# cboin1996/avddpg

Measured on AMD Instinct MI355X. Metric: env-steps/sec + DDPG updates/sec, 4096x5-vehicle platoons, higher is better.
Workload: dtype f32-class (fp16 hi+lo operand pairs on the 16-bit matrix cores, f32 accumulate)

## Files before the change

### avddpg_amd/csrc/fsplit.hip

```cpp
#include <type_traits>

#include "fset_common.h"

namespace avd {
namespace fsplit {
using namespace fset;

struct ActorS {
    static constexpr int K = 256, KP = 256, NFT = 8, NKS = 16, LD = 264, NGT = 9, KG = 288;
    static constexpr bool critic = false;
};
struct CriticS {
    static constexpr int K = 304, KP = 320, NFT = 10, NKS = 19, LD = 312, NGT = 10, KG = 320;
    static constexpr bool critic = true;
};
constexpr int NGT_MAX = 10;

template <int I, int N, class F>
__device__ __forceinline__ void static_for(F&& f) {
    if constexpr (I < N) {
        f(std::integral_constant<int, I>{});
        static_for<I + 1, N>(f);
    }
}
// ... 634 lines not shown
#endif
    if (watch >= 0x7f800000u) atomicOr(p.bad, 1);
    if (BOTH) {
#pragma unroll
        for (int o = 1; o < 32; o <<= 1) {
            Dacc += __shfl_xor(Dacc, o), Lacc += __shfl_xor(Lacc, o);
            Dacc2 += __shfl_xor(Dacc2, o), Lacc2 += __shfl_xor(Lacc2, o);
        }
#pragma unroll
        for (int o = 1; o < 64; o <<= 1) gmax = fmaxf(gmax, __shfl_xor(gmax, o));
        if (lane == 0) {
            const long slot = (long)blockIdx.x * 8 + w;
            p.part_m[slot] = gmax;
            p.part_s[slot * 2] = Dacc, p.part_s[slot * 2 + 1] = Lacc;
            p.part_s2[slot * 2] = Dacc2, p.part_s2[slot * 2 + 1] = Lacc2;
        }
    }
}

struct SeedArgs {
    int n_agents, n_sets;
    const float *dmu, *tz;
    float high;
    float *g3, *part_m, *part_s;
};
__global__ __launch_bounds__(NT) void actor_seed_kernel(const SeedArgs p) {
    const int tid = threadIdx.x, w = tid >> 6, lane = tid & 63;
    const int set = blockIdx.x % p.n_sets, j0 = blockIdx.x / p.n_sets, J = gridDim.x / p.n_sets, P = p.n_agents / p.n_sets;
    float gmax = 0.f, D = 0.f;
    for (int pi = j0 + w * J; pi < P; pi += 8 * J) {
        const long ri = (long)(pi * p.n_sets + set) * TILE + lane;
        const float t = p.tz[ri], g = p.dmu[ri] * p.high * (1.f - t * t);
        p.g3[ri] = g;
        gmax = fmaxf(gmax, fabsf(g));
        D += g;
    }
#pragma unroll
    for (int o = 1; o < 64; o <<= 1) gmax = fmaxf(gmax, __shfl_xor(gmax, o)), D += __shfl_xor(D, o);
    if (lane == 0) {
        p.part_m[(long)blockIdx.x * 8 + w] = gmax;
        p.part_s[((long)blockIdx.x * 8 + w) * 2] = D, p.part_s[((long)blockIdx.x * 8 + w) * 2 + 1] = 0.f;
    }
}

__device__ __forceinline__ float set_gscale(const float* part_m, int set, int n_sets, int J, float* red) {
    const int tid = threadIdx.x;
    float m = 0.f;
    for (int i = tid; i < J * 8; i += NT) m = fmaxf(m, part_m[((long)(i >> 3) * n_sets + set) * 8 + (i & 7)]);
#pragma unroll
    for (int o = 1; o < 64; o <<= 1) m = fmaxf(m, __shfl_xor(m, o));
    if ((tid & 63) == 0) red[tid >> 6] = m;
    __syncthreads();
    m = fmaxf(fmaxf(fmaxf(red[0], red[1]), fmaxf(red[2], red[3])), fmaxf(fmaxf(red[4], red[5]), fmaxf(red[6], red[7])));
    int e = 0;
    if (m > 0.f && !not_finite(m)) (void)frexpf(m, &e);
    const int k = e > 100 ? -100 : (e < -100 ? 100 : -e);
    return __uint_as_float(__builtin_amdgcn_readfirstlane(__float_as_uint(ldexpf(1.f, k))));
}

__device__ __forceinline__ unsigned mask_pair(unsigned d, int j, unsigned mj) { return __umul24(d & (0x10001u << j), mj); }
__device__ __forceinline__ void mask_chunk16(unsigned w, int c, unsigned m, uint4& lo, uint4& hi) {
    const unsigned d = w >> (8 * (c & 1));
    lo.x = mask_pair(d, 0, m), lo.y = mask_pair(d, 1, m >> 1), lo.z = mask_pair(d, 2, m >> 2), lo.w = mask_pair(d, 3, m >> 3);
    hi.x = mask_pair(d, 4, m >> 4), hi.y = mask_pair(d, 5, m >> 5), hi.z = mask_pair(d, 6, m >> 6), hi.w = mask_pair(d, 7, m >> 7);
}
__device__ __forceinline__ unsigned mask_one(float g3, bool signed_) { return signed_ && g3 < 0.f ? 0xbc00u : 0x3c00u; }

struct DwArgs {
    NetP net;
    int n_agents, n_sets;
    const float* x;
    const float* act;
    const float* g3;
    const float* part_m;
    const unsigned* sm;
    float* partG;
    int abl;
    unsigned long long* stamp;
};
template <int S, class NET>
__global__ __launch_bounds__(NT) void dw_kernel(const DwArgs p) {
    constexpr int KG = NET::KG, LDZ = 160;
    constexpr int XC = NET::critic ? 2 : 1;
    constexpr bool SGN = !NET::critic;
    __shared__ __attribute__((aligned(16))) unsigned short sgn16[2][TILE];
    __shared__ __attribute__((aligned(16))) f16 smimg[2][TILE * LDZ];
    __shared__ __attribute__((aligned(16))) f16x8 fq[2][TILE * 2];
    __shared__ __attribute__((aligned(16))) f16x8 fa[2][TILE * 2];
    __shared__ float gred[8];
    const int tid = threadIdx.x, w = tid >> 6, lane = tid & 63, r = lane & 31, h = lane >> 5;
    const int set = blockIdx.x % p.n_sets, j0 = blockIdx.x / p.n_sets, J = gridDim.x / p.n_sets, P = p.n_agents / p.n_sets;
    const float gsc = set_gscale(p.part_m, set, p.n_sets, J, gred);
    const f16x8* wf1 = p.net.wf1h + (long)set * NGT_MAX * 64 + lane;
    const int xt = NET::critic ? 8 + (w >> 2) : 8, xrh = NET::critic ? (w >> 1) & 1 : (w >> 2) & 1, xc0 = NET::critic ? 2 * (w & 1) : (w & 3);
    const f16x8 wf0 = wf1[64 * w], wfx = wf1[64 * xt];
    f32x16 G0[4], G1[XC];
    const f32x16 zero16 = {};
#pragma unroll
    for (int c = 0; c < 4; ++c) G0[c] = zero16;
#pragma unroll
    for (int c = 0; c < XC; ++c) G1[c] = zero16;

    const int srow = tid >> 3, sch = tid & 7, frow = tid >> 1, fh = tid & 1;
    unsigned ma = 0, mb = 0;
    float sx[4] = {0.f, 0.f, 0.f, 0.f}, sg = 0.f, sa = 0.f, ga = 0.f, gb = 0.f;
    auto fetch_m = [&](int pl, unsigned& m, float& g) {
        const long ri = (long)(((FSPLIT_ABL(p.abl) & 1) ? j0 : pl) * p.n_sets + set) * TILE + srow;
        m = p.sm[ri * 4 + (sch >> 1)];
        if (NET::critic) g = p.g3[ri];
    };
    auto fetch_x = [&](int pl) {
        if (pl >= P || tid >= 2 * TILE) return;
        const long ri = (long)(pl * p.n_sets + set) * TILE + frow;
        load_x<S>(p.x, ri, sx);
        sg = p.g3[ri];
        if (NET::critic) sa = p.act[ri];
    };
    auto stage = [&](int pl, int buf, unsigned m, float g) {
        if (pl >= P) return;
        uint4* dst = (uint4*)(smimg[buf] + srow * LDZ + 16 * sch);
        mask_chunk16(m, sch, mask_one(g, NET::critic), dst[0], dst[1]);
        if (tid < 2 * TILE) {
            const float g = fabsf(sg) * gsc;
            fq[buf][tid] = make_xg(g * sx[0], g * sx[1], g * sx[2], g * sx[3], g, fh);
            if (NET::critic) fa[buf][tid] = make_xg(g * sa, 0.f, 0.f, 0.f, g, fh);
            if (SGN && fh == 0) sgn16[buf][frow] = sg < 0.f ? 0x8000 : 0;
        }
    };
    const int g4 = lane >> 4, q = (lane & 15) >> 2, pp = lane & 3;
    typedef _Float16 f16x4 __attribute__((ext_vector_type(4)));
    auto read_tr = [&](const f16* at) {
        return __builtin_bit_cast(f16x4, __builtin_amdgcn_ds_read_tr16_b64_v4bf16((__attribute__((address_space(3))) bf16x4*)at));
    };
    auto read_b = [&](int buf, int e, int s, f16x8 (&bfr)[4]) {
#pragma unroll
        for (int c = 0; c < 4; ++c)
#pragma unroll
            for (int hf = 0; hf < 2; ++hf) {
                const int R0 = 32 * e + 16 * s + 8 * hf + 4 * (g4 >> 1);
                const f16x4 t = read_tr(smimg[buf] + (R0 + q) * LDZ + 32 * c + 16 * (g4 & 1) + 4 * pp);
#pragma unroll
                for (int j = 0; j < 4; ++j) bfr[c][4 * hf + j] = t[j];
            }
    };
    auto split16e = [&](const f32x16& p1, unsigned (&qh)[8], unsigned (&ql)[8], int buf, int e) {
        if (FSPLIT_ABL(p.abl) & 4) {
#pragma unroll
            for (int m = 0; m < 8; ++m) qh[m] = __float_as_uint(p1[2 * m]), ql[m] = __float_as_uint(p1[2 * m + 1]);
            return;
        }
#pragma unroll
        for (int m = 0; m < 8; ++m) split2h(relu(p1[2 * m]), relu(p1[2 * m + 1]), qh[m], ql[m]);
        if (SGN) {
#pragma unroll
            for (int qd = 0; qd < 4; ++qd) {
                const uint2 sw = *(const uint2*)((const unsigned*)sgn16[buf] + 16 * e + 4 * qd + 2 * h);
                qh[2 * qd] ^= sw.x, ql[2 * qd] ^= sw.x, qh[2 * qd + 1] ^= sw.y, ql[2 * qd + 1] ^= sw.y;
            }
        }
    };
    auto compute = [&](int buf) {
        unsigned ah[8], al[8], bh[8], bl[8];
        split16e(mfmah(fq[buf][r * 2 + h], wf0, zero16), ah, al, buf, 0);
        __builtin_amdgcn_sched_barrier(0);
        {
            const f32x16 p1 = mfmah(fq[buf][(32 + r) * 2 + h], wf0, zero16);
#pragma unroll
            for (int s = 0; s < 2; ++s) {
                f16x8 bfr[4];
                read_b(buf, 0, s, bfr);
                const f16x8 hi = fragh(ah[4 * s], ah[4 * s + 1], ah[4 * s + 2], ah[4 * s + 3]);
                const f16x8 lo = fragh(al[4 * s], al[4 * s + 1], al[4 * s + 2], al[4 * s + 3]);
#pragma unroll
                for (int c = 0; c < 4; ++c) G0[c] = mfmah(hi, bfr[c], G0[c]), G0[c] = mfmah(lo, bfr[c], G0[c]);
            }
            split16e(p1, bh, bl, buf, 1);
            __builtin_amdgcn_sched_group_barrier(0x008, 1, 0);
#pragma unroll
            for (int s = 0; s < 2; ++s) {
                __builtin_amdgcn_sched_group_barrier(0x100, 8, 0);
#pragma unroll
                for (int i = 0; i < 8; ++i) {
                    __builtin_amdgcn_sched_group_barrier(0x008, 1, 0);
                    __builtin_amdgcn_sched_group_barrier(0x002, SGN ? 4 : 3, 0);
                }
            }
            __builtin_amdgcn_sched_barrier(0);
        }
        {
            const f16x8 xin = NET::critic ? fa[buf][(32 * xrh + r) * 2 + h] : fq[buf][(32 * xrh + r) * 2 + h];
            const f32x16 px = mfmah(xin, wfx, zero16);
#pragma unroll
            for (int s = 0; s < 2; ++s) {
                f16x8 bfr[4];
                read_b(buf, 1, s, bfr);
                const f16x8 hi = fragh(bh[4 * s], bh[4 * s + 1], bh[4 * s + 2], bh[4 * s + 3]);
                const f16x8 lo = fragh(bl[4 * s], bl[4 * s + 1], bl[4 * s + 2], bl[4 * s + 3]);
#pragma unroll
                for (int c = 0; c < 4; ++c) G0[c] = mfmah(hi, bfr[c], G0[c]), G0[c] = mfmah(lo, bfr[c], G0[c]);
            }
            split16e(px, ah, al, buf, xrh);
            __builtin_amdgcn_sched_group_barrier(0x008, 1, 0);
#pragma unroll
            for (int s = 0; s < 2; ++s) {
                __builtin_amdgcn_sched_group_barrier(0x100, 8, 0);
#pragma unroll
                for (int i = 0; i < 8; ++i) {
                    __builtin_amdgcn_sched_group_barrier(0x008, 1, 0);
                    __builtin_amdgcn_sched_group_barrier(0x002, SGN ? 4 : 3, 0);
                }
            }
            __builtin_amdgcn_sched_barrier(0);
        }
#pragma unroll
        for (int s = 0; s < 2; ++s) {
            const f16x8 hi = fragh(ah[4 * s], ah[4 * s + 1], ah[4 * s + 2], ah[4 * s + 3]);
            const f16x8 lo = fragh(al[4 * s], al[4 * s + 1], al[4 * s + 2], al[4 * s + 3]);
#pragma unroll
            for (int c = 0; c < XC; ++c) {
                f16x8 bx;
#pragma unroll
                for (int hf = 0; hf < 2; ++hf) {
                    const int R0 = 32 * xrh + 16 * s + 8 * hf + 4 * (g4 >> 1);
                    const f16x4 t = read_tr(smimg[buf] + (R0 + q) * LDZ + 32 * (xc0 + c) + 16 * (g4 & 1) + 4 * pp);
#pragma unroll
                    for (int j = 0; j < 4; ++j) bx[4 * hf + j] = t[j];
                }
                G1[c] = mfmah(hi, bx, G1[c]);
                G1[c] = mfmah(lo, bx, G1[c]);
            }
        }
    };
    if (j0 < P) fetch_m(j0, ma, ga);
    fetch_x(j0);
    if (j0 + J < P) fetch_m(j0 + J, mb, gb);
    stage(j0, 0, ma, ga);
    __syncthreads();
#ifdef AVD_STAMP
    unsigned long long tacc[4] = {0, 0, 0, 0}, tlast = __builtin_amdgcn_s_memtime();
#define STAMP(i) { const unsigned long long t_ = __builtin_amdgcn_s_memtime(); tacc[i] += t_ - tlast; tlast = t_; }
#else
#define STAMP(i)
#endif
    for (int pi = j0; pi < P; pi += 2 * J) {
        fetch_x(pi + J);
        if (pi + 2 * J < P) fetch_m(pi + 2 * J, ma, ga);
        STAMP(0);
        compute(0);
        STAMP(1);
        stage(pi + J, 1, mb, gb);
        STAMP(2);
        if (!(FSPLIT_ABL(p.abl) & 2)) __syncthreads();
        STAMP(3);
        if (pi + J < P) {
            fetch_x(pi + 2 * J);
            if (pi + 3 * J < P) fetch_m(pi + 3 * J, mb, gb);
            STAMP(0);
            compute(1);
            STAMP(1);
            stage(pi + 2 * J, 0, ma, ga);
            STAMP(2);
            if (!(FSPLIT_ABL(p.abl) & 2)) __syncthreads();
            STAMP(3);
        }
    }
#ifdef AVD_STAMP
    if (p.stamp && blockIdx.x == 16 && lane == 0)
        for (int i = 0; i < 4; ++i) p.stamp[w * 8 + i] = tacc[i];
#endif
    const float dsc = 1.f / (gsc * S1);
    float* comb = (float*)&smimg[0][0];
    const int cidx = NET::critic ? 2 * (w >> 2) + (w & 1) : (w & 3);
    if (xrh == 1) {
#pragma unroll
        for (int c = 0; c < XC; ++c)
#pragma unroll
            for (int k = 0; k < 16; ++k) comb[((cidx * XC + c) * 16 + k) * 64 + lane] = G1[c][k];
    }
    __syncthreads();
#pragma unroll
    for (int c = 0; c < 4; ++c) {
        float* dst = p.partG + ((long)blockIdx.x * KG + 32 * w) * H2 + 32 * c + r;
#pragma unroll
        for (int k = 0; k < 16; ++k) dst[(long)acc_row(k, h) * H2] = G0[c][k] * dsc;
    }
    if (xrh == 0) {
#pragma unroll
        for (int c = 0; c < XC; ++c) {
            float* dst = p.partG + ((long)blockIdx.x * KG + 32 * xt) * H2 + 32 * (xc0 + c) + r;
#pragma unroll
            for (int k = 0; k < 16; ++k) dst[(long)acc_row(k, h) * H2] = (G1[c][k] + comb[((cidx * XC + c) * 16 + k) * 64 + lane]) * dsc;
        }
    }
}

struct DxArgs {
    NetP net;
    int n_agents, n_sets;
    const f16x8* xfh;
    const float* act;
    int L_cWa, L_cba;
    const float* g3;
    const float* part_m;
    const unsigned* sm;
    int unsigned_mask;
    float* partV;
    int abl;
    unsigned long long* stamp;
};
template <int S, class NET>
__global__ __launch_bounds__(NT) void dx_kernel(const DxArgs p) {
    constexpr int KP = NET::KP, LDZ = 136;
    constexpr float VSH = 1.f / 32.f;
    __shared__ __attribute__((aligned(16))) f16 smimg[2][TILE * LDZ];
    __shared__ __attribute__((aligned(16))) f16 xt[2][2][32 * 32];
    __shared__ __attribute__((aligned(16))) float g3s[2][TILE];
    __shared__ float gred[8];
    const int tid = threadIdx.x, w = __builtin_amdgcn_readfirstlane(tid >> 6), lane = tid & 63, r = lane & 31, h = lane >> 5, ft = w;
    const int set = blockIdx.x % p.n_sets, j0 = blockIdx.x / p.n_sets, J = gridDim.x / p.n_sets, P = p.n_agents / p.n_sets;
    const f32x16 zero16 = {};
    const float gsc = set_gscale(p.part_m, set, p.n_sets, J, gred);
    f16x8 wch[8], wcl[8];
    {
        const long at = ((long)set * KP + 32 * ft + r) * H2 + 8 * h;
#pragma unroll
        for (int s = 0; s < 8; ++s) wch[s] = *(const f16x8*)(p.net.Wchi + at + 16 * s), wcl[s] = *(const f16x8*)(p.net.Wclo + at + 16 * s);
    }
    const float swc = __uint_as_float(__builtin_amdgcn_readfirstlane(__float_as_uint(p.net.vec[(long)set * VEC + 2 * H2 + 2])));
    const float gv = gsc * VSH, vs = gsc * swc * VSH;
    const f16x8 wf = p.net.wf1h[((long)set * NGT_MAX + ft) * 64 + lane];
    f32x16 V = zero16;
    for (int i = tid; i < 2 * 2 * 32 * 32; i += NT) {
        const int k = (i >> 5) & 31;
        (&xt[0][0][0])[i] = (f16)(k == 8 ? 1.f : 0.f);
    }
    const int srow = tid >> 3, sch = tid & 7;
    unsigned dm = 0;
    float gn = 0.f, gs = 0.f;
    auto fetch = [&](int agent) {
        if (FSPLIT_ABL(p.abl) & 1) agent = j0 * p.n_sets + set;
        dm = p.sm[((long)agent * TILE + srow) * 4 + (sch >> 1)];
        if (NET::critic) gs = p.g3[(long)agent * TILE + srow];
        if (tid < TILE) gn = p.g3[(long)agent * TILE + tid];
    };
    auto stage = [&](int buf) {
        uint4* dst = (uint4*)(smimg[buf] + srow * LDZ + 16 * sch);
        mask_chunk16(dm, sch, mask_one(gs, NET::critic), dst[0], dst[1]);
        if (tid < TILE) g3s[buf][tid] = (p.unsigned_mask ? gn : fabsf(gn)) * gv;
    };
    f16x8 xfn0 = {}, xfn1 = {};
    auto fetch_x = [&](int agent) {
        xfn0 = p.xfh[((long)agent * TILE + r) * 2 + h];
        xfn1 = p.xfh[((long)agent * TILE + 32 + r) * 2 + h];
    };
    auto stage_x = [&](int buf) {
        if (w < 2 && h == 0) {
            f16x8 src = xfn0;
            if (w == 1) src = xfn1;
            asm volatile("" : "+v"(src));
#pragma unroll
            for (int k = 0; k < 8; ++k) xt[buf][w][k * 32 + r] = src[k];
        }
    };
    __syncthreads();
    if (j0 < P) fetch(j0 * p.n_sets + set), fetch_x(j0 * p.n_sets + set), stage(0), stage_x(0);
    __syncthreads();
#ifdef AVD_STAMP
    unsigned long long dacc[4] = {0, 0, 0, 0}, dlast = __builtin_amdgcn_s_memtime();
#define DXSTAMP(i) { const unsigned long long t_ = __builtin_amdgcn_s_memtime(); dacc[i] += t_ - dlast; dlast = t_; }
#else
#define DXSTAMP(i)
#endif
    int buf = 0;
    for (int pi = j0; pi < P; pi += J, buf ^= 1) {
        const bool more = pi + J < P;
        const f16x8 xf[2] = {xfn0, xfn1};
        if (more) fetch((pi + J) * p.n_sets + set), fetch_x((pi + J) * p.n_sets + set);
        DXSTAMP(0);
        auto read_a = [&](int e, f16x8 (&smf)[8]) {
            const f16* arow = smimg[buf] + (32 * e + r) * LDZ + 8 * h;
#pragma unroll
            for (int s = 0; s < 8; ++s) smf[s] = *(const f16x8*)(arow + 16 * s);
        };
        typedef _Float16 f16x4 __attribute__((ext_vector_type(4)));
        auto read_img = [&](const f16* img, f16x8 (&xb)[2]) {
#pragma unroll
            for (int s = 0; s < 2; ++s) {
                const f16x4 lo = *(const f16x4*)(img + r * 32 + 16 * s + 4 * h);
                const f16x4 hi = *(const f16x4*)(img + r * 32 + 16 * s + 8 + 4 * h);
#pragma unroll
                for (int j = 0; j < 4; ++j) xb[s][j] = lo[j], xb[s][4 + j] = hi[j];
            }
        };
        auto backward = [&](int e, const f32x16& dc, const f32x16& p1, unsigned (&vh)[8], unsigned (&vl)[8]) {
            if (FSPLIT_ABL(p.abl) & 4) {
#pragma unroll
                for (int m = 0; m < 8; ++m) vh[m] = __float_as_uint(dc[2 * m]) ^ __float_as_uint(p1[2 * m]), vl[m] = __float_as_uint(dc[2 * m + 1]);
                return;
            }
#pragma unroll
            for (int g = 0; g < 4; ++g) {
                const float4 gq = *(const float4*)(&g3s[buf][32 * e + 8 * g + 4 * h]);
                const float gg[4] = {gq.x, gq.y, gq.z, gq.w};
                float dm[4];
#pragma unroll
                for (int j = 0; j < 4; ++j) {
                    const int k = 4 * g + j;
                    dm[j] = p1[k] > 0.f ? dc[k] * gg[j] : 0.f;
                }
                split2h(dm[0], dm[1], vh[2 * g], vl[2 * g]);
                split2h(dm[2], dm[3], vh[2 * g + 1], vl[2 * g + 1]);
            }
        };
        f16x8 smf[8], xb0[2], xb1[2];
        unsigned vh0[8], vl0[8], vh1[8], vl1[8];
        read_a(0, smf);
        f32x16 dc0 = zero16;
#pragma unroll
        for (int s = 0; s < 8; ++s) dc0 = mfmah(smf[s], wch[s], dc0), dc0 = mfmah(smf[s], wcl[s], dc0);
        const f32x16 p10 = mfmah(xf[0], wf, zero16);
        __builtin_amdgcn_sched_barrier(0);
        read_a(1, smf);
        read_img(xt[buf][0], xb0);
        f32x16 dc1 = zero16;
#pragma unroll
        for (int s = 0; s < 8; ++s) dc1 = mfmah(smf[s], wch[s], dc1), dc1 = mfmah(smf[s], wcl[s], dc1);
        const f32x16 p11 = mfmah(xf[1], wf, zero16);
        backward(0, dc0, p10, vh0, vl0);
        __builtin_amdgcn_sched_group_barrier(0x100, 12, 0);
#pragma unroll
        for (int i = 0; i < 17; ++i) {
            __builtin_amdgcn_sched_group_barrier(0x008, 1, 0);
            __builtin_amdgcn_sched_group_barrier(0x002, 5, 0);
            __builtin_amdgcn_sched_group_barrier(0x100, 1, 0);
        }
        __builtin_amdgcn_sched_barrier(0);
        read_img(xt[buf][1], xb1);
#pragma unroll
        for (int s = 0; s < 2; ++s) {
            V = mfmah(fragh(vh0[4 * s], vh0[4 * s + 1], vh0[4 * s + 2], vh0[4 * s + 3]), xb0[s], V);
            V = mfmah(fragh(vl0[4 * s], vl0[4 * s + 1], vl0[4 * s + 2], vl0[4 * s + 3]), xb0[s], V);
        }
        backward(1, dc1, p11, vh1, vl1);
#pragma unroll
        for (int s = 0; s < 2; ++s) {
            V = mfmah(fragh(vh1[4 * s], vh1[4 * s + 1], vh1[4 * s + 2], vh1[4 * s + 3]), xb1[s], V);
            V = mfmah(fragh(vl1[4 * s], vl1[4 * s + 1], vl1[4 * s + 2], vl1[4 * s + 3]), xb1[s], V);
        }
        DXSTAMP(1);
        if (more) stage(buf ^ 1), stage_x(buf ^ 1);
        DXSTAMP(2);
        if (!(FSPLIT_ABL(p.abl) & 2)) __syncthreads();
        DXSTAMP(3);
    }
#ifdef AVD_STAMP
    if (p.stamp && blockIdx.x == 16 && lane == 0)
        for (int i = 0; i < 4; ++i) p.stamp[w * 8 + i] = dacc[i];
#endif
    const float ivs = 1.f / vs;
    if (r < 16) {
        float* pv = p.partV + ((long)blockIdx.x * KP + 32 * ft) * 16 + r;
#pragma unroll
        for (int k = 0; k < 16; ++k) pv[(long)acc_row(k, h) * 16] = V[k] * ivs;
    }
}

template <int S>
__global__ __launch_bounds__(NT) void dxa_kernel(const DxArgs p) {
    typedef CriticS NET;
    constexpr int KP = NET::KP;
    constexpr float VSH = 1.f / 32.f;
    __shared__ __attribute__((aligned(16))) float ga[8][2][2][32];
    __shared__ float comb[8][64][2];
    __shared__ float gred[8];
    const int tid = threadIdx.x, w = __builtin_amdgcn_readfirstlane(tid >> 6), lane = tid & 63, r = lane & 31, h = lane >> 5;
    const int rh = w & 1, ftl = (w >> 1) & 1, par = w >> 2;
    const int set = blockIdx.x % p.n_sets, j0 = blockIdx.x / p.n_sets, J = gridDim.x / p.n_sets, P = p.n_agents / p.n_sets;
    const f32x16 zero16 = {};
    const int ft = 8 + ftl, f = 32 * ftl + r;
    const float gsc = set_gscale(p.part_m, set, p.n_sets, J, gred);
    f16x8 wch[8], wcl[8];
    {
        const long at = ((long)set * KP + 32 * ft + r) * H2 + 8 * h;
#pragma unroll
        for (int s = 0; s < 8; ++s) wch[s] = *(const f16x8*)(p.net.Wchi + at + 16 * s), wcl[s] = *(const f16x8*)(p.net.Wclo + at + 16 * s);
    }
    const float swc = __uint_as_float(__builtin_amdgcn_readfirstlane(__float_as_uint(p.net.vec[(long)set * VEC + 2 * H2 + 2])));
    const float gv = gsc * VSH, vs = gsc * swc * VSH;
    const float* th = p.net.th + (long)set * p.net.th_stride;
    const float wa = f < HA ? th[p.L_cWa + f] : 0.f, ba = f < HA ? th[p.L_cba + f] : 0.f;
    float Sa = 0.f, Sb = 0.f;
    const int ntile = j0 < P ? (P - j0 + J - 1) / J : 0;
    uint4 mA = {}, mB = {};
    float gA = 0.f, aA = 0.f, gB = 0.f, aB = 0.f;
#define DXA_FETCH(k_, m_, g_, a_)                                                                                   \
    {                                                                                                               \
        const long r0_ = (long)((j0 + (k_) * J) * p.n_sets + set) * TILE + 32 * rh;                                 \
        m_ = *(const uint4*)(p.sm + (r0_ + r) * 4);                                                                 \
        g_ = p.g3[r0_ + r], a_ = p.act[r0_ + r];                                                                    \
    }
#define DXA_PUT(buf_, g_, a_)                                                                                       \
    {                                                                                                               \
        if (h == 0) ga[w][buf_][0][r] = fabsf(g_) * gv, ga[w][buf_][1][r] = a_;                                     \
        __builtin_amdgcn_fence(__ATOMIC_RELEASE, "wavefront");                                                      \
        __builtin_amdgcn_wave_barrier();                                                                            \
    }
    auto unit = [&](int buf, const uint4 mw, float g) {
        f32x16 dc = zero16;
        const unsigned m = mask_one(g, true);
        const unsigned mwt[4] = {mw.x >> (4 * h), mw.y >> (4 * h), mw.z >> (4 * h), mw.w >> (4 * h)};
#pragma unroll
        for (int s = 0; s < 8; ++s) {
            const unsigned d = mwt[s >> 1] >> (8 * (s & 1));
            const f16x8 af = fragh(mask_pair(d, 0, m), mask_pair(d, 1, m >> 1), mask_pair(d, 2, m >> 2), mask_pair(d, 3, m >> 3));
            dc = mfmah(af, wch[s], dc), dc = mfmah(af, wcl[s], dc);
        }
        float sa = 0.f, sb = 0.f;
#pragma unroll
        for (int q = 0; q < 4; ++q) {
            const float4 gq = *(const float4*)(&ga[w][buf][0][8 * q + 4 * h]), aq = *(const float4*)(&ga[w][buf][1][8 * q + 4 * h]);
            const float gg[4] = {gq.x, gq.y, gq.z, gq.w}, av[4] = {aq.x, aq.y, aq.z, aq.w};
#pragma unroll
            for (int j = 0; j < 4; ++j) {
                const float m = fmaf(av[j], wa, ba) > 0.f ? dc[4 * q + j] * gg[j] : 0.f;
                sa = fmaf(m, av[j], sa);
                sb += m;
            }
        }
        Sa += sa, Sb += sb;
        __builtin_amdgcn_fence(__ATOMIC_ACQ_REL, "wavefront");
        __builtin_amdgcn_wave_barrier();
    };
    if (par < ntile) DXA_FETCH(par, mA, gA, aA);
    if (par + 2 < ntile) DXA_FETCH(par + 2, mB, gB, aB);
    for (int k = par; k < ntile; k += 4) {
        DXA_PUT(0, gA, aA);
// ... 53 lines not shown
        pl.Whi[i] = take(sizeof(f16) * (size_t)n_sets * H2 * K), pl.Wlo[i] = take(sizeof(f16) * (size_t)n_sets * H2 * K);
        pl.vec[i] = take(sizeof(float) * (size_t)n_sets * VEC);
        pl.wf1h[i] = take(16 * (size_t)n_sets * NGT_MAX * 64);
        if (i < 2) pl.Wchi[i] = take(sizeof(f16) * (size_t)n_sets * KP * H2), pl.Wclo[i] = take(sizeof(f16) * (size_t)n_sets * KP * H2);
    }
    pl.wap = take(4 * (size_t)n_sets * 48);
    const size_t rows = (size_t)n_agents * TILE;
    pl.a2 = take(4 * rows), pl.y = take(4 * rows), pl.mu = take(4 * rows), pl.dmu = take(4 * rows), pl.g3 = take(4 * rows);
    pl.sm = take(16 * rows);
    pl.sma = take(16 * rows);
    pl.tz = take(4 * rows);
    pl.t1p = take(2 * 4 * (size_t)n_sets * CriticS::K * H2), pl.s2raw = take(2 * 4 * (size_t)n_sets * H2);
    pl.xfs = take(32 * rows), pl.xfs2 = take(32 * rows);
    for (int i = 0; i < 2; ++i) {
        const int KP = i ? CriticS::KP : ActorS::KP, KG = i ? CriticS::KG : ActorS::KG;
        pl.partM[i] = take(4 * (size_t)pl.grid * 8);
        pl.partV[i] = take(4 * (size_t)pl.grid * KP * 16);
        pl.partG[i] = take(4 * (size_t)pl.grid * KG * H2);
    }
    for (int i = 0; i < 3; ++i) pl.partHs[i] = take(4 * (size_t)pl.grid * 8 * 2);
    pl.bad = take(sizeof(int) + sizeof(unsigned) * 4 * (size_t)n_sets * 2);
    pl.total = o;
    return pl;
}
static int check_shape(const avd_mlp_layout* L, int n_agents, int n_sets, const char* who) {
    AVD_REQUIRE(L, "%s: null layout", who);
    if (L->H1 != H1 || L->H2 != H2 || L->Ha != HA || L->A != 1 || (L->S != 3 && L->S != 4) || L->B != TILE) {
        set_error("%s: serves the reference widths only (layer1 256, layer2 128, action layer 48, A = 1, S in {3, 4}, B = 64); "
                  "got H1=%d H2=%d Ha=%d A=%d S=%d B=%d (avd_learn_shared_bf16 takes other widths)",
                  who, L->H1, L->H2, L->Ha, L->A, L->S, L->B);
        return AVD_E_UNSUPPORTED;
    }
    AVD_REQUIRE(n_sets > 0 && n_sets <= 64 && n_agents > 0 && n_agents % n_sets == 0, "%s: n_agents=%d n_sets=%d", who, n_agents,
                n_sets);
    return AVD_OK;
}

enum Phase { PH_CRITIC = 1, PH_ACTOR = 2, PH_BOTH = 3 };
template <int S>
static int run(int phases, const avd_mlp_layout& L, int n_agents, int n_sets, const float* theta, const float* stats, const float* theta_t,
               const float* stats_t, const float* s, const float* a, const float* r, const float* s2, const float* aw, float gamma,
               float high, float* grads, float* losses, unsigned char* ws, const Plan& pl, hipStream_t st) {
    PrepArgs pa;
    pa.L = L, pa.S = S, pa.theta = theta, pa.stats = stats, pa.theta_t = theta_t, pa.stats_t = stats_t;
    pa.wap = (unsigned*)(ws + pl.wap), pa.bad = (int*)(ws + pl.bad), pa.smax = (unsigned*)(ws + pl.bad + sizeof(int));
    NetP net[4];
    for (int i = 0; i < 4; ++i) {
        const bool critic = i & 1, target = i >= 2;
        pa.Whi[i] = (f16*)(ws + pl.Whi[i]), pa.Wlo[i] = (f16*)(ws + pl.Wlo[i]), pa.vec[i] = (float*)(ws + pl.vec[i]);
        pa.wf1h[i] = (f16x8*)(ws + pl.wf1h[i]);
        pa.Wchi[i] = i < 2 ? (f16*)(ws + pl.Wchi[i]) : nullptr, pa.Wclo[i] = i < 2 ? (f16*)(ws + pl.Wclo[i]) : nullptr;
        NetP& n = net[i];
        n.th = (target ? theta_t : theta) + (critic ? L.actor_size : 0), n.th_stride = L.theta_size;
        n.Whi = pa.Whi[i], n.Wlo = pa.Wlo[i], n.Wchi = pa.Wchi[i], n.Wclo = pa.Wclo[i], n.wf1h = pa.wf1h[i], n.vec = pa.vec[i];
        n.wap = pa.wap;
    }
    const int P = n_agents / n_sets;
    const float inv_n = 1.0f / ((float)P * TILE);
    const long nrows = (long)n_agents * TILE;
    f16x8 *xfs = (f16x8*)(ws + pl.xfs), *xfs2 = (f16x8*)(ws + pl.xfs2);
    int* bad = (int*)(ws + pl.bad);
    float *a2 = (float*)(ws + pl.a2), *y = (float*)(ws + pl.y), *mu = (float*)(ws + pl.mu), *dmu = (float*)(ws + pl.dmu);
    float* g3 = (float*)(ws + pl.g3);
    unsigned *sm = (unsigned*)(ws + pl.sm), *sma = (unsigned*)(ws + pl.sma);
    auto F = [&](size_t off) { return (float*)(ws + off); };
    const dim3 grid(pl.grid), block(NT);
    HeadArgs h;
    h.n_agents = n_agents, h.n_sets = n_sets, h.gamma = gamma, h.high = high, h.inv_n = inv_n, h.aw = aw, h.sm = sm, h.g3 = g3, h.dmu = dmu;
    h.act2 = nullptr, h.part_s2 = nullptr, h.stamp = nullptr, h.bad = bad, h.part_m = nullptr, h.tz = F(pl.tz), h.abl = 0;
    if (const char* e = AVD_DIAG_ENV("FSPLIT_ABL")) h.abl = atoi(e);
    auto head = [&](auto kern, int ni, const f16x8* x, const float* act, const float* rr, const float* yin, float* out, float* part_s) {
        h.net = net[ni], h.xf = x, h.act = act, h.r = rr, h.yin = yin, h.out = out, h.part_s = part_s;
        hipLaunchKernelGGL(kern, grid, block, 0, st, h);
    };
    DwArgs dw;
    dw.n_agents = n_agents, dw.n_sets = n_sets, dw.sm = sm, dw.g3 = g3, dw.x = s, dw.stamp = nullptr, dw.abl = 0;
    if (const char* e = AVD_DIAG_ENV("FSPLIT_ABL")) dw.abl = atoi(e);
#ifdef AVD_STAMP
    static unsigned long long* d_stamp = nullptr;
    if (!d_stamp) (void)hipMalloc(&d_stamp, 128 * 8);
    dw.stamp = d_stamp;
#endif
    DxArgs dx;
    dx.n_agents = n_agents, dx.n_sets = n_sets, dx.sm = sm, dx.g3 = g3, dx.xfh = xfs, dx.stamp = nullptr, dx.L_cWa = dx.L_cba = 0, dx.unsigned_mask = 0;
    dx.abl = dw.abl;
#ifdef AVD_STAMP
    dx.stamp = d_stamp;
#endif
    FinArgs fa;
    fa.L = L, fa.n_sets = n_sets, fa.J = pl.J, fa.S = S, fa.nrh = 1, fa.theta = theta, fa.stats = stats, fa.grads = grads, fa.losses = losses;
    fa.inv_n = inv_n, fa.partLa = F(pl.partHs[2]), fa.bad = bad;
    for (int i = 0; i < 2; ++i)
        fa.partH[i] = nullptr, fa.partHs[i] = F(pl.partHs[i]), fa.partU[i] = nullptr, fa.partV[i] = F(pl.partV[i]),
        fa.partG[i] = F(pl.partG[i]), fa.c3[i] = F(pl.vec[i]);
    fa.t1_from_g[0] = fa.t1_from_g[1] = 1, fa.t1p = F(pl.t1p), fa.s2raw = F(pl.s2raw);
    if (phases & PH_CRITIC) {
        if (hipMemsetAsync(ws + pl.bad, 0, sizeof(int) + sizeof(unsigned) * 4 * (size_t)n_sets * 2, st) != hipSuccess)
            return check_launch("avd_learn_set_split: memset");
        hipLaunchKernelGGL(scale_kernel, dim3(4, n_sets, SCALE_SLICES), dim3(256), 0, st, pa);
        hipLaunchKernelGGL(prep_kernel, dim3(H2, 4, n_sets), dim3(320), 0, st, pa);
        hipLaunchKernelGGL(prep1_kernel, dim3(NGT_MAX, 4, n_sets), dim3(64), 0, st, pa);
        PackArgs pk;
        pk.x[0] = s, pk.extra[0] = a, pk.outh[0] = xfs, pk.x[1] = s2, pk.extra[1] = r, pk.outh[1] = xfs2, pk.rows = nrows, pk.bad = bad;
        hipLaunchKernelGGL(pack_x_kernel<S>, dim3((unsigned)((2 * nrows + 255) / 256), 2), dim3(256), 0, st, pk);
        head(head_kernel<S, ActorS, OUT_TANH>, 2, xfs2, nullptr, nullptr, nullptr, a2, nullptr);
        head(head_kernel<S, CriticS, OUT_TD>, 3, xfs2, a2, r, nullptr, y, nullptr);
        h.sm = sma;
        head(head_kernel<S, ActorS, OUT_TANH_SAVE>, 0, xfs, nullptr, nullptr, nullptr, mu, nullptr);
        h.sm = sm;
        h.act2 = mu, h.part_s2 = F(pl.partHs[2]), h.part_m = F(pl.partM[1]);
        head(head_kernel<S, CriticS, HEAD_BOTH>, 1, xfs, a, nullptr, y, nullptr, F(pl.partHs[1]));
        dw.net = net[1], dw.act = a, dw.partG = F(pl.partG[1]), dw.part_m = F(pl.partM[1]);
        hipLaunchKernelGGL((dw_kernel<S, CriticS>), grid, block, 0, st, dw);
        dx.net = net[1], dx.partV = F(pl.partV[1]), dx.act = a, dx.part_m = F(pl.partM[1]);
        hipLaunchKernelGGL((dx_kernel<S, CriticS>), grid, block, 0, st, dx);
        dx.L_cWa = L.cWa, dx.L_cba = L.cba;
        hipLaunchKernelGGL((dxa_kernel<S>), grid, block, 0, st, dx);
        if (phases == PH_CRITIC) launch_finalize(fa, st, 1, 1);
    }
    if (phases & PH_ACTOR) {
        SeedArgs sd;
        sd.n_agents = n_agents, sd.n_sets = n_sets, sd.dmu = dmu, sd.tz = F(pl.tz), sd.high = high, sd.g3 = g3, sd.part_m = F(pl.partM[0]),
        sd.part_s = F(pl.partHs[0]);
        hipLaunchKernelGGL(actor_seed_kernel, grid, block, 0, st, sd);
        dw.sm = sma, dx.sm = sma;
        dw.net = net[0], dw.act = nullptr, dw.partG = F(pl.partG[0]), dw.part_m = F(pl.partM[0]);
        hipLaunchKernelGGL((dw_kernel<S, ActorS>), grid, block, 0, st, dw);
        dx.net = net[0], dx.partV = F(pl.partV[0]), dx.act = nullptr, dx.part_m = F(pl.partM[0]), dx.L_cWa = dx.L_cba = 0, dx.unsigned_mask = 1;
        hipLaunchKernelGGL((dx_kernel<S, ActorS>), grid, block, 0, st, dx);
        if (phases == PH_ACTOR) launch_finalize(fa, st, 0, 1);
        else launch_finalize(fa, st, 0, 2);
    }
    return check_launch("avd_learn_set_split");
}

}
}

using namespace avd;

namespace avd { namespace fsplit {
constexpr long MFMA_PER_TILE = 2 * (200 + 238 + 200 + 314)
                               + 8 * (2 + 32 + 1 + 2 * 2 * 2)
                               + 8 * (2 + 32 + 1 + 2 * 1 * 2)
                               + 2 * 8 * (32 + 2 + 8)
                               + 4 * 16;
static_assert(MFMA_PER_TILE == 3296, "update DESIGN.md 3.4 and the count above together");
}}
extern "C" int avd_learn_set_split_mfma_count(const avd_mlp_layout* lay, int n_agents, int n_sets, unsigned long long* mfma_32x32x16) {
    int rc = fsplit::check_shape(lay, n_agents, n_sets, "avd_learn_set_split_mfma_count");
    if (rc) return rc;
    AVD_REQUIRE(mfma_32x32x16, "avd_learn_set_split_mfma_count: null pointer");
    *mfma_32x32x16 = (unsigned long long)fsplit::MFMA_PER_TILE * (unsigned long long)n_agents;
    return AVD_OK;
}

extern "C" int avd_learn_set_split_workspace(const avd_mlp_layout* lay, int n_agents, int n_sets, size_t* bytes) {
    int rc = fsplit::check_shape(lay, n_agents, n_sets, "avd_learn_set_split_workspace");
    if (rc) return rc;
    AVD_REQUIRE(bytes, "avd_learn_set_split_workspace: null pointer");
    *bytes = fsplit::make_plan(n_agents, n_sets).total;
    return AVD_OK;
}

static int split_entry(int phases, const char* who, const avd_mlp_layout* lay, int n_agents, int n_sets, const float* theta, const float* stats,
                       const float* theta_t, const float* stats_t, const float* s, const float* a, const float* r, const float* s2,
                       const float* agent_weight, float gamma, float high, float* grads, float* losses, void* workspace,
                       size_t workspace_bytes, void* stream) {
    int rc = fsplit::check_shape(lay, n_agents, n_sets, who);
    if (rc) return rc;
    const bool cr = phases & fsplit::PH_CRITIC;
    AVD_REQUIRE(theta && stats && s && grads && workspace && (!cr || (theta_t && stats_t && a && r && s2)), "%s: null pointer", who);
    const fsplit::Plan pl = fsplit::make_plan(n_agents, n_sets);
    AVD_REQUIRE(workspace_bytes >= pl.total, "%s: workspace %zu B < %zu B", who, workspace_bytes, pl.total);
    if (cr && hipMemsetAsync(grads, 0, sizeof(float) * (size_t)n_sets * lay->theta_size, (hipStream_t)stream) != hipSuccess)
        return check_launch("avd_learn_set_split: hipMemsetAsync(grads)");
    if (lay->S == 4)
        return fsplit::run<4>(phases, *lay, n_agents, n_sets, theta, stats, theta_t, stats_t, s, a, r, s2, agent_weight, gamma, high, grads,
                              losses, (unsigned char*)workspace, pl, (hipStream_t)stream);
    return fsplit::run<3>(phases, *lay, n_agents, n_sets, theta, stats, theta_t, stats_t, s, a, r, s2, agent_weight, gamma, high, grads, losses,
                          (unsigned char*)workspace, pl, (hipStream_t)stream);
}

extern "C" int avd_learn_set_split_f16x3(const avd_mlp_layout* lay, int n_agents, int n_sets, const float* theta, const float* stats,
                                          const float* theta_t, const float* stats_t, const float* s, const float* a, const float* r,
                                          const float* s2, const float* agent_weight, float gamma, float high, float* grads,
                                          float* losses, void* workspace, size_t workspace_bytes, void* stream) {
    return split_entry(fsplit::PH_BOTH, "avd_learn_set_split_f16x3", lay, n_agents, n_sets, theta, stats, theta_t, stats_t, s, a, r, s2,
                       agent_weight, gamma, high, grads, losses, workspace, workspace_bytes, stream);
}

extern "C" int avd_learn_set_split_bf16x3(const avd_mlp_layout* lay, int n_agents, int n_sets, const float* theta, const float* stats,
                                          const float* theta_t, const float* stats_t, const float* s, const float* a, const float* r,
                                          const float* s2, const float* agent_weight, float gamma, float high, float* grads,
                                          float* losses, void* workspace, size_t workspace_bytes, void* stream) {
    return avd_learn_set_split_f16x3(lay, n_agents, n_sets, theta, stats, theta_t, stats_t, s, a, r, s2, agent_weight, gamma, high, grads,
                                     losses, workspace, workspace_bytes, stream);
}

extern "C" int avd_learn_set_split_critic(const avd_mlp_layout* lay, int n_agents, int n_sets, const float* theta, const float* stats,
                                          const float* theta_t, const float* stats_t, const float* s, const float* a, const float* r,
                                          const float* s2, const float* agent_weight, float gamma, float high, float* grads,
                                          float* losses, void* workspace, size_t workspace_bytes, void* stream) {
    return split_entry(fsplit::PH_CRITIC, "avd_learn_set_split_critic", lay, n_agents, n_sets, theta, stats, theta_t, stats_t, s, a, r, s2,
                       agent_weight, gamma, high, grads, losses, workspace, workspace_bytes, stream);
}

extern "C" int avd_learn_set_split_actor(const avd_mlp_layout* lay, int n_agents, int n_sets, const float* theta, const float* stats,
                                         const float* s, float high, float* grads, void* workspace, size_t workspace_bytes, void* stream) {
    return split_entry(fsplit::PH_ACTOR, "avd_learn_set_split_actor", lay, n_agents, n_sets, theta, stats, nullptr, nullptr, s, nullptr, nullptr,
                       nullptr, nullptr, 0.f, high, grads, nullptr, workspace, workspace_bytes, stream);
// ... 2 lines not shown
```

Measured before the change: 2.019 million.

## Software-pipeline dx kernel across tiles and fold actor sign into mask staging

The dx kernel is restructured so the second half of each tile's backward pass and V-product run overlapped with the next tile's dc products. Staging now uses a three-slot ring for xt/g3s, with a one-ahead prefetch of mask and x data. In dw, the per-row sign XOR on the split operands is removed and the sign is instead folded into the staged mask image (signed ±1 mask for the actor). Mask staging for the next buffer is moved inside compute, with scheduling hints interleaving it with the MFMAs. Costs are more shared memory, more complex prologue/epilogue logic, and a sign-convention change whose correctness depends on mask_one semantics.

```diff
diff --git a/avddpg_amd/csrc/fsplit.hip b/avddpg_amd/csrc/fsplit.hip
--- a/avddpg_amd/csrc/fsplit.hip
+++ b/avddpg_amd/csrc/fsplit.hip
@@ -740,8 +740,6 @@
 __global__ __launch_bounds__(NT) void dw_kernel(const DwArgs p) {
     constexpr int KG = NET::KG, LDZ = 160;
     constexpr int XC = NET::critic ? 2 : 1;
-    constexpr bool SGN = !NET::critic;
-    __shared__ __attribute__((aligned(16))) unsigned short sgn16[2][TILE];
     __shared__ __attribute__((aligned(16))) f16 smimg[2][TILE * LDZ];
     __shared__ __attribute__((aligned(16))) f16x8 fq[2][TILE * 2];
     __shared__ __attribute__((aligned(16))) f16x8 fa[2][TILE * 2];
@@ -765,7 +763,7 @@
     auto fetch_m = [&](int pl, unsigned& m, float& g) {
         const long ri = (long)(((FSPLIT_ABL(p.abl) & 1) ? j0 : pl) * p.n_sets + set) * TILE + srow;
         m = p.sm[ri * 4 + (sch >> 1)];
-        if (NET::critic) g = p.g3[ri];
+        g = p.g3[ri];
     };
     auto fetch_x = [&](int pl) {
         if (pl >= P || tid >= 2 * TILE) return;
@@ -774,15 +772,16 @@
         sg = p.g3[ri];
         if (NET::critic) sa = p.act[ri];
     };
-    auto stage = [&](int pl, int buf, unsigned m, float g) {
+    auto stage_m = [&](int buf, unsigned m, float g) {
+        uint4* dst = (uint4*)(smimg[buf] + srow * LDZ + 16 * sch);
+        mask_chunk16(m, sch, mask_one(g, true), dst[0], dst[1]);
+    };
+    auto stage_x = [&](int pl, int buf) {
         if (pl >= P) return;
-        uint4* dst = (uint4*)(smimg[buf] + srow * LDZ + 16 * sch);
-        mask_chunk16(m, sch, mask_one(g, NET::critic), dst[0], dst[1]);
         if (tid < 2 * TILE) {
             const float g = fabsf(sg) * gsc;
             fq[buf][tid] = make_xg(g * sx[0], g * sx[1], g * sx[2], g * sx[3], g, fh);
             if (NET::critic) fa[buf][tid] = make_xg(g * sa, 0.f, 0.f, 0.f, g, fh);
-            if (SGN && fh == 0) sgn16[buf][frow] = sg < 0.f ? 0x8000 : 0;
         }
     };
     const int g4 = lane >> 4, q = (lane & 15) >> 2, pp = lane & 3;
@@ -801,7 +800,7 @@
                 for (int j = 0; j < 4; ++j) bfr[c][4 * hf + j] = t[j];
             }
     };
-    auto split16e = [&](const f32x16& p1, unsigned (&qh)[8], unsigned (&ql)[8], int buf, int e) {
+    auto split16e = [&](const f32x16& p1, unsigned (&qh)[8], unsigned (&ql)[8]) {
         if (FSPLIT_ABL(p.abl) & 4) {
 #pragma unroll
             for (int m = 0; m < 8; ++m) qh[m] = __float_as_uint(p1[2 * m]), ql[m] = __float_as_uint(p1[2 * m + 1]);
@@ -809,17 +808,10 @@
         }
 #pragma unroll
         for (int m = 0; m < 8; ++m) split2h(relu(p1[2 * m]), relu(p1[2 * m + 1]), qh[m], ql[m]);
-        if (SGN) {
-#pragma unroll
-            for (int qd = 0; qd < 4; ++qd) {
-                const uint2 sw = *(const uint2*)((const unsigned*)sgn16[buf] + 16 * e + 4 * qd + 2 * h);
-                qh[2 * qd] ^= sw.x, ql[2 * qd] ^= sw.x, qh[2 * qd + 1] ^= sw.y, ql[2 * qd + 1] ^= sw.y;
-            }
-        }
-    };
-    auto compute = [&](int buf) {
+    };
+    auto compute = [&](int buf, unsigned m, float g) {
         unsigned ah[8], al[8], bh[8], bl[8];
-        split16e(mfmah(fq[buf][r * 2 + h], wf0, zero16), ah, al, buf, 0);
+        split16e(mfmah(fq[buf][r * 2 + h], wf0, zero16), ah, al);
         __builtin_amdgcn_sched_barrier(0);
         {
             const f32x16 p1 = mfmah(fq[buf][(32 + r) * 2 + h], wf0, zero16);
@@ -832,7 +824,7 @@
 #pragma unroll
                 for (int c = 0; c < 4; ++c) G0[c] = mfmah(hi, bfr[c], G0[c]), G0[c] = mfmah(lo, bfr[c], G0[c]);
             }
-            split16e(p1, bh, bl, buf, 1);
+            split16e(p1, bh, bl);
             __builtin_amdgcn_sched_group_barrier(0x008, 1, 0);
 #pragma unroll
             for (int s = 0; s < 2; ++s) {
@@ -840,7 +832,7 @@
 #pragma unroll
                 for (int i = 0; i < 8; ++i) {
                     __builtin_amdgcn_sched_group_barrier(0x008, 1, 0);
-                    __builtin_amdgcn_sched_group_barrier(0x002, SGN ? 4 : 3, 0);
+                    __builtin_amdgcn_sched_group_barrier(0x002, 3, 0);
                 }
             }
             __builtin_amdgcn_sched_barrier(0);
@@ -857,7 +849,7 @@
 #pragma unroll
                 for (int c = 0; c < 4; ++c) G0[c] = mfmah(hi, bfr[c], G0[c]), G0[c] = mfmah(lo, bfr[c], G0[c]);
             }
-            split16e(px, ah, al, buf, xrh);
+            split16e(px, ah, al);
             __builtin_amdgcn_sched_group_barrier(0x008, 1, 0);
 #pragma unroll
             for (int s = 0; s < 2; ++s) {
@@ -865,11 +857,12 @@
 #pragma unroll
                 for (int i = 0; i < 8; ++i) {
                     __builtin_amdgcn_sched_group_barrier(0x008, 1, 0);
-                    __builtin_amdgcn_sched_group_barrier(0x002, SGN ? 4 : 3, 0);
+                    __builtin_amdgcn_sched_group_barrier(0x002, 3, 0);
                 }
             }
             __builtin_amdgcn_sched_barrier(0);
         }
+        stage_m(buf ^ 1, m, g);
 #pragma unroll
         for (int s = 0; s < 2; ++s) {
             const f16x8 hi = fragh(ah[4 * s], ah[4 * s + 1], ah[4 * s + 2], ah[4 * s + 3]);
@@ -888,11 +881,19 @@
                 G1[c] = mfmah(lo, bx, G1[c]);
             }
         }
+        __builtin_amdgcn_sched_group_barrier(0x100, 4 * XC, 0);
+#pragma unroll
+        for (int i = 0; i < 4 * XC; ++i) {
+            __builtin_amdgcn_sched_group_barrier(0x008, 1, 0);
+            __builtin_amdgcn_sched_group_barrier(0x002, 6, 0);
+        }
+        __builtin_amdgcn_sched_group_barrier(0x200, 2, 0);
+        __builtin_amdgcn_sched_barrier(0);
     };
     if (j0 < P) fetch_m(j0, ma, ga);
     fetch_x(j0);
     if (j0 + J < P) fetch_m(j0 + J, mb, gb);
-    stage(j0, 0, ma, ga);
+    stage_m(0, ma, ga), stage_x(j0, 0);
     __syncthreads();
 #ifdef AVD_STAMP
     unsigned long long tacc[4] = {0, 0, 0, 0}, tlast = __builtin_amdgcn_s_memtime();
@@ -904,9 +905,9 @@
         fetch_x(pi + J);
         if (pi + 2 * J < P) fetch_m(pi + 2 * J, ma, ga);
         STAMP(0);
-        compute(0);
+        compute(0, mb, gb);
         STAMP(1);
-        stage(pi + J, 1, mb, gb);
+        stage_x(pi + J, 1);
         STAMP(2);
         if (!(FSPLIT_ABL(p.abl) & 2)) __syncthreads();
         STAMP(3);
@@ -914,9 +915,9 @@
             fetch_x(pi + 2 * J);
             if (pi + 3 * J < P) fetch_m(pi + 3 * J, mb, gb);
             STAMP(0);
-            compute(1);
+            compute(1, ma, ga);
             STAMP(1);
-            stage(pi + 2 * J, 0, ma, ga);
+            stage_x(pi + 2 * J, 0);
             STAMP(2);
             if (!(FSPLIT_ABL(p.abl) & 2)) __syncthreads();
             STAMP(3);
@@ -961,7 +962,6 @@
     const float* g3;
     const float* part_m;
     const unsigned* sm;
-    int unsigned_mask;
     float* partV;
     int abl;
     unsigned long long* stamp;
@@ -971,8 +971,8 @@
     constexpr int KP = NET::KP, LDZ = 136;
     constexpr float VSH = 1.f / 32.f;
     __shared__ __attribute__((aligned(16))) f16 smimg[2][TILE * LDZ];
-    __shared__ __attribute__((aligned(16))) f16 xt[2][2][32 * 32];
-    __shared__ __attribute__((aligned(16))) float g3s[2][TILE];
+    __shared__ __attribute__((aligned(16))) f16 xt[3][2][32 * 32];
+    __shared__ __attribute__((aligned(16))) float g3s[3][TILE];
     __shared__ float gred[8];
     const int tid = threadIdx.x, w = __builtin_amdgcn_readfirstlane(tid >> 6), lane = tid & 63, r = lane & 31, h = lane >> 5, ft = w;
     const int set = blockIdx.x % p.n_sets, j0 = blockIdx.x / p.n_sets, J = gridDim.x / p.n_sets, P = p.n_agents / p.n_sets;
@@ -988,128 +988,160 @@
     const float gv = gsc * VSH, vs = gsc * swc * VSH;
     const f16x8 wf = p.net.wf1h[((long)set * NGT_MAX + ft) * 64 + lane];
     f32x16 V = zero16;
-    for (int i = tid; i < 2 * 2 * 32 * 32; i += NT) {
+    for (int i = tid; i < 3 * 2 * 32 * 32; i += NT) {
         const int k = (i >> 5) & 31;
         (&xt[0][0][0])[i] = (f16)(k == 8 ? 1.f : 0.f);
     }
     const int srow = tid >> 3, sch = tid & 7;
     unsigned dm = 0;
     float gn = 0.f, gs = 0.f;
-    auto fetch = [&](int agent) {
-        if (FSPLIT_ABL(p.abl) & 1) agent = j0 * p.n_sets + set;
-        dm = p.sm[((long)agent * TILE + srow) * 4 + (sch >> 1)];
-        if (NET::critic) gs = p.g3[(long)agent * TILE + srow];
-        if (tid < TILE) gn = p.g3[(long)agent * TILE + tid];
-    };
-    auto stage = [&](int buf) {
+    auto fetch = [&](int pl) {
+        if (FSPLIT_ABL(p.abl) & 1) pl = j0;
+        const long agent = (long)pl * p.n_sets + set;
+        dm = p.sm[(agent * TILE + srow) * 4 + (sch >> 1)];
+        if (NET::critic) gs = p.g3[agent * TILE + srow];
+        if (tid < TILE) gn = p.g3[agent * TILE + tid];
+    };
+    auto stage = [&](int buf, int slot) {
         uint4* dst = (uint4*)(smimg[buf] + srow * LDZ + 16 * sch);
         mask_chunk16(dm, sch, mask_one(gs, NET::critic), dst[0], dst[1]);
-        if (tid < TILE) g3s[buf][tid] = (p.unsigned_mask ? gn : fabsf(gn)) * gv;
+        if (tid < TILE) g3s[slot][tid] = (NET::critic ? fabsf(gn) : gn) * gv;
     };
     f16x8 xfn0 = {}, xfn1 = {};
-    auto fetch_x = [&](int agent) {
-        xfn0 = p.xfh[((long)agent * TILE + r) * 2 + h];
-        xfn1 = p.xfh[((long)agent * TILE + 32 + r) * 2 + h];
-    };
-    auto stage_x = [&](int buf) {
+    auto fetch_x = [&](int pl) {
+        const long agent = (long)pl * p.n_sets + set;
+        xfn0 = p.xfh[(agent * TILE + r) * 2 + h];
+        xfn1 = p.xfh[(agent * TILE + 32 + r) * 2 + h];
+    };
+    auto stage_x = [&](int slot) {
         if (w < 2 && h == 0) {
             f16x8 src = xfn0;
             if (w == 1) src = xfn1;
             asm volatile("" : "+v"(src));
 #pragma unroll
-            for (int k = 0; k < 8; ++k) xt[buf][w][k * 32 + r] = src[k];
-        }
-    };
-    __syncthreads();
-    if (j0 < P) fetch(j0 * p.n_sets + set), fetch_x(j0 * p.n_sets + set), stage(0), stage_x(0);
-    __syncthreads();
+            for (int k = 0; k < 8; ++k) xt[slot][w][k * 32 + r] = src[k];
+        }
+    };
 #ifdef AVD_STAMP
     unsigned long long dacc[4] = {0, 0, 0, 0}, dlast = __builtin_amdgcn_s_memtime();
 #define DXSTAMP(i) { const unsigned long long t_ = __builtin_amdgcn_s_memtime(); dacc[i] += t_ - dlast; dlast = t_; }
 #else
 #define DXSTAMP(i)
 #endif
-    int buf = 0;
-    for (int pi = j0; pi < P; pi += J, buf ^= 1) {
-        const bool more = pi + J < P;
-        const f16x8 xf[2] = {xfn0, xfn1};
-        if (more) fetch((pi + J) * p.n_sets + set), fetch_x((pi + J) * p.n_sets + set);
+    auto read_a = [&](int buf, int e, f16x8 (&smf)[8]) {
+        const f16* arow = smimg[buf] + (32 * e + r) * LDZ + 8 * h;
+#pragma unroll
+        for (int s = 0; s < 8; ++s) smf[s] = *(const f16x8*)(arow + 16 * s);
+    };
+    typedef _Float16 f16x4 __attribute__((ext_vector_type(4)));
+    auto read_img = [&](const f16* img, f16x8 (&xb)[2]) {
+#pragma unroll
+        for (int s = 0; s < 2; ++s) {
+            const f16x4 lo = *(const f16x4*)(img + r * 32 + 16 * s + 4 * h);
+            const f16x4 hi = *(const f16x4*)(img + r * 32 + 16 * s + 8 + 4 * h);
+#pragma unroll
+            for (int j = 0; j < 4; ++j) xb[s][j] = lo[j], xb[s][4 + j] = hi[j];
+        }
+    };
+    auto dc_product = [&](const f16x8 (&smf)[8]) {
+        f32x16 dc = zero16;
+#pragma unroll
+        for (int s = 0; s < 8; ++s) dc = mfmah(smf[s], wch[s], dc), dc = mfmah(smf[s], wcl[s], dc);
+        return dc;
+    };
+    auto backward = [&](int slot, int e, const f32x16& dc, const f32x16& p1, unsigned (&vh)[8], unsigned (&vl)[8]) {
+        if (FSPLIT_ABL(p.abl) & 4) {
+#pragma unroll
+            for (int m = 0; m < 8; ++m) vh[m] = __float_as_uint(dc[2 * m]) ^ __float_as_uint(p1[2 * m]), vl[m] = __float_as_uint(dc[2 * m + 1]);
+            return;
+        }
+#pragma unroll
+        for (int g = 0; g < 4; ++g) {
+            const float4 gq = *(const float4*)(&g3s[slot][32 * e + 8 * g + 4 * h]);
+            const float gg[4] = {gq.x, gq.y, gq.z, gq.w};
+            float dm[4];
+#pragma unroll
+            for (int j = 0; j < 4; ++j) {
+                const int k = 4 * g + j;
+                dm[j] = p1[k] > 0.f ? dc[k] * gg[j] : 0.f;
+            }
+            split2h(dm[0], dm[1], vh[2 * g], vl[2 * g]);
+            split2h(dm[2], dm[3], vh[2 * g + 1], vl[2 * g + 1]);
+        }
+    };
+    auto v_product = [&](const unsigned (&vh)[8], const unsigned (&vl)[8], const f16x8 (&xb)[2]) {
+#pragma unroll
+        for (int s = 0; s < 2; ++s) {
+            V = mfmah(fragh(vh[4 * s], vh[4 * s + 1], vh[4 * s + 2], vh[4 * s + 3]), xb[s], V);
+            V = mfmah(fragh(vl[4 * s], vl[4 * s + 1], vl[4 * s + 2], vl[4 * s + 3]), xb[s], V);
+        }
+    };
+    f16x8 xf0, xf1;
+    f32x16 dc1 = zero16, p11 = zero16;
+    auto iteration = [&](auto has_prev_c, int pi, int buf, int slot) {
+        constexpr bool has_prev = decltype(has_prev_c)::value;
+        const int pslot = slot == 0 ? 2 : slot - 1, nslot = slot == 2 ? 0 : slot + 1;
+        const int nn = pi + 2 * J < P ? pi + 2 * J : (pi + J < P ? pi + J : pi);
         DXSTAMP(0);
-        auto read_a = [&](int e, f16x8 (&smf)[8]) {
-            const f16* arow = smimg[buf] + (32 * e + r) * LDZ + 8 * h;
-#pragma unroll
-            for (int s = 0; s < 8; ++s) smf[s] = *(const f16x8*)(arow + 16 * s);
-        };
-        typedef _Float16 f16x4 __attribute__((ext_vector_type(4)));
-        auto read_img = [&](const f16* img, f16x8 (&xb)[2]) {
-#pragma unroll
-            for (int s = 0; s < 2; ++s) {
-                const f16x4 lo = *(const f16x4*)(img + r * 32 + 16 * s + 4 * h);
-                const f16x4 hi = *(const f16x4*)(img + r * 32 + 16 * s + 8 + 4 * h);
-#pragma unroll
-                for (int j = 0; j < 4; ++j) xb[s][j] = lo[j], xb[s][4 + j] = hi[j];
-            }
-        };
-        auto backward = [&](int e, const f32x16& dc, const f32x16& p1, unsigned (&vh)[8], unsigned (&vl)[8]) {
-            if (FSPLIT_ABL(p.abl) & 4) {
-#pragma unroll
-                for (int m = 0; m < 8; ++m) vh[m] = __float_as_uint(dc[2 * m]) ^ __float_as_uint(p1[2 * m]), vl[m] = __float_as_uint(dc[2 * m + 1]);
-                return;
-            }
-#pragma unroll
-            for (int g = 0; g < 4; ++g) {
-                const float4 gq = *(const float4*)(&g3s[buf][32 * e + 8 * g + 4 * h]);
-                const float gg[4] = {gq.x, gq.y, gq.z, gq.w};
-                float dm[4];
-#pragma unroll
-                for (int j = 0; j < 4; ++j) {
-                    const int k = 4 * g + j;
-                    dm[j] = p1[k] > 0.f ? dc[k] * gg[j] : 0.f;
-                }
-                split2h(dm[0], dm[1], vh[2 * g], vl[2 * g]);
-                split2h(dm[2], dm[3], vh[2 * g + 1], vl[2 * g + 1]);
-            }
-        };
         f16x8 smf[8], xb0[2], xb1[2];
         unsigned vh0[8], vl0[8], vh1[8], vl1[8];
-        read_a(0, smf);
-        f32x16 dc0 = zero16;
-#pragma unroll
-        for (int s = 0; s < 8; ++s) dc0 = mfmah(smf[s], wch[s], dc0), dc0 = mfmah(smf[s], wcl[s], dc0);
-        const f32x16 p10 = mfmah(xf[0], wf, zero16);
+        read_a(buf, 0, smf);
+        const f32x16 dc0 = dc_product(smf);
+        const f32x16 p10 = mfmah(xf0, wf, zero16);
+        if constexpr (has_prev) {
+            read_img(xt[pslot][1], xb1);
+            backward(pslot, 1, dc1, p11, vh1, vl1);
+            __builtin_amdgcn_sched_group_barrier(0x100, 12, 0);
+#pragma unroll
+            for (int i = 0; i < 17; ++i) {
+                __builtin_amdgcn_sched_group_barrier(0x008, 1, 0);
+                __builtin_amdgcn_sched_group_barrier(0x002, 5, 0);
+                __builtin_amdgcn_sched_group_barrier(0x100, 1, 0);
+            }
+        }
         __builtin_amdgcn_sched_barrier(0);
-        read_a(1, smf);
-        read_img(xt[buf][0], xb0);
-        f32x16 dc1 = zero16;
-#pragma unroll
-        for (int s = 0; s < 8; ++s) dc1 = mfmah(smf[s], wch[s], dc1), dc1 = mfmah(smf[s], wcl[s], dc1);
-        const f32x16 p11 = mfmah(xf[1], wf, zero16);
-        backward(0, dc0, p10, vh0, vl0);
-        __builtin_amdgcn_sched_group_barrier(0x100, 12, 0);
-#pragma unroll
-        for (int i = 0; i < 17; ++i) {
+        DXSTAMP(1);
+        if constexpr (has_prev) v_product(vh1, vl1, xb1);
+        read_a(buf, 1, smf);
+        read_img(xt[slot][0], xb0);
+        dc1 = dc_product(smf);
+        p11 = mfmah(xf1, wf, zero16);
+        backward(slot, 0, dc0, p10, vh0, vl0);
+        stage(buf ^ 1, nslot);
+        stage_x(nslot);
+        xf0 = xfn0, xf1 = xfn1;
+        fetch(nn), fetch_x(nn);
+        __builtin_amdgcn_sched_group_barrier(0x100, 16, 0);
+#pragma unroll
+        for (int i = 0; i < (has_prev ? 21 : 17); ++i) {
             __builtin_amdgcn_sched_group_barrier(0x008, 1, 0);
-            __builtin_amdgcn_sched_group_barrier(0x002, 5, 0);
-            __builtin_amdgcn_sched_group_barrier(0x100, 1, 0);
+            __builtin_amdgcn_sched_group_barrier(0x002, 6, 0);
+            __builtin_amdgcn_sched_group_barrier(0x200, 1, 0);
         }
         __builtin_amdgcn_sched_barrier(0);
-        read_img(xt[buf][1], xb1);
-#pragma unroll
-        for (int s = 0; s < 2; ++s) {
-            V = mfmah(fragh(vh0[4 * s], vh0[4 * s + 1], vh0[4 * s + 2], vh0[4 * s + 3]), xb0[s], V);
-            V = mfmah(fragh(vl0[4 * s], vl0[4 * s + 1], vl0[4 * s + 2], vl0[4 * s + 3]), xb0[s], V);
-        }
-        backward(1, dc1, p11, vh1, vl1);
-#pragma unroll
-        for (int s = 0; s < 2; ++s) {
-            V = mfmah(fragh(vh1[4 * s], vh1[4 * s + 1], vh1[4 * s + 2], vh1[4 * s + 3]), xb1[s], V);
-            V = mfmah(fragh(vl1[4 * s], vl1[4 * s + 1], vl1[4 * s + 2], vl1[4 * s + 3]), xb1[s], V);
-        }
-        DXSTAMP(1);
-        if (more) stage(buf ^ 1), stage_x(buf ^ 1);
+        v_product(vh0, vl0, xb0);
         DXSTAMP(2);
         if (!(FSPLIT_ABL(p.abl) & 2)) __syncthreads();
         DXSTAMP(3);
+    };
+    __syncthreads();
+    if (j0 < P) {
+        fetch(j0), fetch_x(j0), stage(0, 0), stage_x(0);
+        xf0 = xfn0, xf1 = xfn1;
+        const int n1 = j0 + J < P ? j0 + J : j0;
+        fetch(n1), fetch_x(n1);
+    }
+    __syncthreads();
+    if (j0 < P) {
+        iteration(std::false_type{}, j0, 0, 0);
+        int buf = 1, slot = 1, pi = j0 + J;
+        for (; pi < P; pi += J, buf ^= 1, slot = slot == 2 ? 0 : slot + 1) iteration(std::true_type{}, pi, buf, slot);
+        const int pslot = slot == 0 ? 2 : slot - 1;
+        f16x8 xb1[2];
+        unsigned vh1[8], vl1[8];
+        read_img(xt[pslot][1], xb1);
+        backward(pslot, 1, dc1, p11, vh1, vl1);
+        v_product(vh1, vl1, xb1);
     }
 #ifdef AVD_STAMP
     if (p.stamp && blockIdx.x == 16 && lane == 0)
@@ -1329,7 +1361,7 @@
     dw.stamp = d_stamp;
 #endif
     DxArgs dx;
-    dx.n_agents = n_agents, dx.n_sets = n_sets, dx.sm = sm, dx.g3 = g3, dx.xfh = xfs, dx.stamp = nullptr, dx.L_cWa = dx.L_cba = 0, dx.unsigned_mask = 0;
+    dx.n_agents = n_agents, dx.n_sets = n_sets, dx.sm = sm, dx.g3 = g3, dx.xfh = xfs, dx.stamp = nullptr, dx.L_cWa = dx.L_cba = 0;
     dx.abl = dw.abl;
 #ifdef AVD_STAMP
     dx.stamp = d_stamp;
@@ -1373,7 +1405,7 @@
         dw.sm = sma, dx.sm = sma;
         dw.net = net[0], dw.act = nullptr, dw.partG = F(pl.partG[0]), dw.part_m = F(pl.partM[0]);
         hipLaunchKernelGGL((dw_kernel<S, ActorS>), grid, block, 0, st, dw);
-        dx.net = net[0], dx.partV = F(pl.partV[0]), dx.act = nullptr, dx.part_m = F(pl.partM[0]), dx.L_cWa = dx.L_cba = 0, dx.unsigned_mask = 1;
+        dx.net = net[0], dx.partV = F(pl.partV[0]), dx.act = nullptr, dx.part_m = F(pl.partM[0]), dx.L_cWa = dx.L_cba = 0;
         hipLaunchKernelGGL((dx_kernel<S, ActorS>), grid, block, 0, st, dx);
         if (phases == PH_ACTOR) launch_finalize(fa, st, 0, 1);
         else launch_finalize(fa, st, 0, 2);
```

Result: faster. 2.094 million (median of 6 runs) (+3.7%).
